# Zaggy1024/RaytracerCore

Hardware: AMD Instinct MI355X
Metric: Mrays/sec (primary+secondary) and samples/sec at 1080p, Cornell box (higher is better)
Workload: dtype f32; 1 GPU; bounce.txt camera 0 1920x1080 x 256 spp per GPU per step; traversal=brute, recursion=10, kernel_build=scene-specialised (hiprtc)

## Files before the change

include/rtcore.h:

```cpp
#ifndef RTCORE_H
#define RTCORE_H

#ifndef __HIPCC_RTC__
#include <stdint.h>
#include <stddef.h>
#endif

#ifdef __cplusplus
extern "C" {
#endif

#define RTCORE_ABI_VERSION 6

typedef enum rt_status {
    RT_OK = 0,
    RT_ERR_ARG = -1,
    RT_ERR_HIP = -2,
    RT_ERR_OOM = -3,
    RT_ERR_NCCL = -4,
    RT_ERR_PARSE = -5,
    RT_ERR_NODEVICE = -6,
    RT_ERR_STATE = -7
} rt_status;

// ... 93 lines not shown
int rt_scene_get_info(const rt_scene* scene, rt_scene_info* info);
void rt_scene_destroy(rt_scene* scene);
int rt_set_bvh_builder(int32_t builder);
int rt_scene_get_build_stats(const rt_scene* scene, double* out, int32_t n);
int rt_set_jit(int32_t on);
int rt_scene_get_jit_error(const rt_scene* scene, char* buf, int32_t cap);
int rt_debug_jit_compile(const char* arch, int32_t grouped, char* log, int32_t cap);
int rt_debug_jit_header(const rt_scene_params* params, const rt_prim* prims, int32_t n_prims, const rt_camera* camera,
                        int32_t grouped, char* buf, int64_t cap);
int rt_scene_check_bvh(rt_scene* scene);
#define RT_LAYOUT_COUNT 10
int rt_debug_brute_layout(const rt_prim* prims, int32_t n_prims, int32_t* out, int32_t n_out);
int rt_debug_item_order(int32_t w, int32_t h, int32_t spp, int32_t chunks, int32_t pool, int32_t band,
                        int32_t band_stride, int32_t band_offset, uint32_t* out, int64_t cap_words, int32_t* info);
int rt_debug_scene_bound(const rt_prim* prims, int32_t n_prims, float* lo, float* hi, float* info);
int rt_debug_ray_log(rt_scene* scene, void* d_log, uint32_t cap, void* d_count);
int rt_debug_vn_rehit(const double* v0, const double* e01, const double* e02, int32_t mirror, double u, double v,
                      const float* dir, int32_t* inside, double* t, double* origin);
int rt_debug_trace_rays(rt_scene* scene, const void* d_rays, uint32_t n, void* d_hits, int32_t waves_per_simd,
                        void* d_stats, void* stream, float* ms);

int rt_render_tile(rt_scene* scene, int32_t x0, int32_t y0, int32_t w, int32_t h, int32_t spp,
                   uint64_t seed, uint64_t sample_base, rt_color* sum_rgb, uint32_t* samples,
                   uint32_t* misses, uint64_t* rays_out);

int rt_render_tile_1spp(rt_scene* scene, int32_t x0, int32_t y0, int32_t w, int32_t h,
                        uint64_t seed, uint64_t sample_index, rt_color* out);

int rt_primary_ids(rt_scene* scene, int32_t x0, int32_t y0, int32_t w, int32_t h, int32_t* ids_out);

// ... 143 lines not shown
```

raytracercore_amd/__init__.py:

```python
from __future__ import annotations

import ctypes as C
import enum
import os
from dataclasses import dataclass
from typing import List, Optional, Sequence, Tuple

import numpy as np

_HERE = os.path.dirname(os.path.abspath(__file__))
LIB_PATH = os.path.join(_HERE, "librtcore_hip.so")
REPO_ROOT = os.path.dirname(_HERE)

RT_OK = 0
ABI_VERSION = 6
RT_PRIM_TRIANGLE, RT_PRIM_SPHERE, RT_PRIM_PLANE = 0, 1, 2
RT_FLAG_MIRROR, RT_FLAG_TWOSIDED, RT_FLAG_INVERT, RT_FLAG_HASNORMALS, RT_FLAG_TRANSFORMED = 1, 2, 4, 8, 16
RT_CAMERA_FRUSTUM, RT_CAMERA_ORTHO = 0, 1
RT_TRAVERSAL_AUTO, RT_TRAVERSAL_BRUTE, RT_TRAVERSAL_BVH, RT_TRAVERSAL_BVH2, RT_TRAVERSAL_GROUPED = 0, 1, 2, 3, 4
RT_BVH_BUILDER_AUTO, RT_BVH_BUILDER_HOST, RT_BVH_BUILDER_GPU = 0, 1, 2
(RT_BOUNCE_SKIPPED, RT_BOUNCE_DIFFUSE, RT_BOUNCE_SPECULAR, RT_BOUNCE_SPECULAR_FAIL, RT_BOUNCE_TRANSMITTED,
 RT_BOUNCE_EMISSION, RT_BOUNCE_PURE_BLACK, RT_BOUNCE_RECURSION_COMPLETE, RT_BOUNCE_MISSED, RT_BOUNCE_DEBUG) = range(10)
BOUNCE_TYPE_NAMES = ("Skipped", "Diffuse", "Specular", "SpecularFail", "Transmitted", "Emission", "PureBlack",
                     "RecursionComplete", "Missed", "Debug")
# ... 187 lines not shown
        "rt_frame_render": (C.c_int, [C.c_void_p, C.c_int32, C.c_uint64, C.c_uint64, P(rt_color), P(C.c_uint32),
                                      P(C.c_uint32), P(C.c_uint64)]),
        "rt_frame_submit": (C.c_int, [C.c_void_p, C.c_int32, C.c_uint64, C.c_uint64]),
        "rt_frame_collect": (C.c_int, [C.c_void_p, P(rt_color), P(C.c_uint32), P(C.c_uint32), P(C.c_uint64)]),
        "rt_frame_inject_fault": (C.c_int, [C.c_void_p, C.c_int32]),
        "rt_frame_destroy": (None, [C.c_void_p]),
        "rt_parse_scene": (C.c_int, [C.c_char_p, P(rt_scene_params), P(rt_prim), P(C.c_int32), P(rt_camera),
                                     P(C.c_int32)]),
        "rt_sample_output": (C.c_int32, [rt_color, C.c_uint32, C.c_uint32, rt_color, C.c_double, C.c_double]),
        "rt_tonemap_device": (C.c_int, [C.c_void_p, C.c_void_p, C.c_void_p, C.c_int32, C.c_int32, rt_color, C.c_double,
                                        C.c_double, C.c_void_p, C.c_void_p]),
        "rt_ref_bvh_export": (C.c_int, [P(rt_prim), C.c_int32, P(C.c_int32), P(C.c_double), P(C.c_int32),
                                        P(C.c_int32)]),
        "rt_debug_item_order": (C.c_int, [C.c_int32] * 8 + [P(C.c_uint32), C.c_int64, P(C.c_int32)]),
        "rt_debug_scene_bound": (C.c_int, [P(rt_prim), C.c_int32, P(C.c_float), P(C.c_float), P(C.c_float)]),
        "rt_debug_ray_log": (C.c_int, [C.c_void_p, C.c_void_p, C.c_uint32, C.c_void_p]),
        "rt_debug_vn_rehit": (C.c_int, [P(C.c_double), P(C.c_double), P(C.c_double), C.c_int32, C.c_double,
                                        C.c_double, P(C.c_float), P(C.c_int32), P(C.c_double), P(C.c_double)]),
        "rt_debug_trace_rays": (C.c_int, [C.c_void_p, C.c_void_p, C.c_uint32, C.c_void_p, C.c_int32, C.c_void_p,
                                          C.c_void_p, P(C.c_float)]),
        "rt_query_rays": (C.c_int, [C.c_void_p, C.c_int32, C.c_void_p, C.c_int64, C.c_void_p]),
        "rt_query_rays_device": (C.c_int, [C.c_void_p, C.c_int32, C.c_void_p, C.c_int64, C.c_void_p, C.c_void_p]),
        "rt_camera_rays": (C.c_int, [P(rt_camera)] + [C.c_int32] * 6 + [C.c_void_p]),
        "rt_select_pixels": (C.c_int, [C.c_void_p, C.c_void_p] + [C.c_int32] * 5 + [C.c_void_p]),
        "rt_select_pixels_device": (C.c_int, [C.c_void_p, C.c_void_p] + [C.c_int32] * 5 + [C.c_void_p, C.c_void_p]),
        "rt_select_rays": (C.c_int, [C.c_void_p, C.c_void_p, C.c_int32, C.c_void_p, C.c_int64, C.c_void_p]),
        "rt_select_rays_device": (C.c_int, [C.c_void_p, C.c_void_p, C.c_int32, C.c_void_p, C.c_int64, C.c_void_p,
                                            C.c_void_p]),
        "rt_debug_select_rays": (C.c_int, [P(rt_prim), C.c_int32, C.c_void_p, C.c_int32, C.c_void_p, C.c_int64,
                                           C.c_void_p]),
# ... 102 lines not shown
    return out[:n], dict(zip(("n_chunks", "chunk", "pool", "n_split"), (int(v) for v in info)))


def scene_bound(prims: Sequence[rt_prim]) -> dict:
    lib = load_library()
    n = len(prims)
    arr = (rt_prim * max(1, n))(*prims)
    lo, hi, info = (C.c_float * 3)(), (C.c_float * 3)(), (C.c_float * 2)()
    state = lib.rt_debug_scene_bound(arr, n, lo, hi, info)
    if state < 0:
        _check(state)
    return {"lo": np.array(lo, np.float32), "hi": np.array(hi, np.float32), "limit": np.float32(info[0]),
            "pad": np.float32(info[1]), "state": int(state)}


def ref_bvh_export(prims: Sequence[rt_prim]) -> Tuple[np.ndarray, np.ndarray, int, int]:
    lib = load_library()
    n = len(prims)
    arr = (rt_prim * max(1, n))(*prims)
    order = np.zeros(max(1, n), np.int32)
    boxes = np.zeros((max(1, 2 * n), 8), np.float64)
    nodes, depth = C.c_int32(0), C.c_int32(0)
    _check(lib.rt_ref_bvh_export(arr, n, order.ctypes.data_as(C.POINTER(C.c_int32)),
                                 boxes.ctypes.data_as(C.POINTER(C.c_double)), C.byref(nodes), C.byref(depth)))
    return order[:n], boxes[:nodes.value], nodes.value, depth.value


def sample_output(sum_rgb: Tuple[float, float, float], samples: int, misses: int,
                  background=(0.0, 0.0, 0.0), background_alpha: float = 0.0, exposure: float = 1.0) -> int:
    lib = load_library()
# ... 114 lines not shown

    def close(self) -> None:
        if self.handle:
            self.lib.rt_scene_destroy(self.handle)
            self.handle = C.c_void_p()

    def __del__(self):
        try:
            self.close()
        except Exception:
            pass

    def set_traversal(self, traversal: int) -> None:
        _check(self.lib.rt_scene_set_traversal(self.handle, traversal))

    def info(self) -> rt_scene_info:
        inf = rt_scene_info()
        _check(self.lib.rt_scene_get_info(self.handle, C.byref(inf)))
        return inf

    def check_bvh(self) -> None:
        _check(self.lib.rt_scene_check_bvh(self.handle))

    def jit_error(self) -> str:
        buf = C.create_string_buffer(4096)
        self.lib.rt_scene_get_jit_error(self.handle, buf, len(buf))
        return buf.value.decode(errors="replace")

    def build_stats(self) -> dict:
        out = (C.c_double * len(BUILD_STAT_NAMES))()
# ... 323 lines not shown
```

raytracercore_amd/csrc/api_debug.hip:

```cpp
#include <cstdlib>
#include <cstring>

#include "rt_scene.h"

namespace {

int n_bvh_prims(const std::vector<HostPrim>& H)
{
    int nb = 0;
    for (const HostPrim& p : H) nb += p.kind != RT_PRIM_PLANE;
    return nb;
}

HostRecords report_records(const std::vector<HostPrim>& H)
{
    const bool host_tree = builder_for(n_bvh_prims(H)) == RT_BVH_BUILDER_HOST;
    return make_host_records(H, host_tree ? grouping_max_leaf(GroupingTree::LayoutReport, (int)H.size(), false) : 0,
                             group_max_default());
}

}

extern "C" {

// ... 422 lines not shown
            set_error("rt_debug_scene_bound: unknown primitive kind at index " + std::to_string(i));
            return RT_ERR_ARG;
        }
    const SceneBound b = make_scene_bound(prepare_prims(prims, n_prims));
    for (int k = 0; k < 3; k++) {
        lo[k] = b.lo[k];
        hi[k] = b.hi[k];
    }
    if (info) {
        info[0] = b.limit;
        info[1] = b.pad;
    }
    return b.empty ? 1 : (b.limit < 0.0f ? 2 : 0);
}

int rt_parse_scene(const char* text, rt_scene_params* params, rt_prim* prims, int32_t* n_prims, rt_camera* cameras,
                   int32_t* n_cameras)
{
    if (!text || !n_prims || !n_cameras) {
        set_error("rt_parse_scene: bad argument");
        return RT_ERR_ARG;
    }
    ParsedScene ps;
    std::string err;
    if (!parse_scene_text(text, ps, err)) {
        set_error(err);
        return RT_ERR_PARSE;
    }
    const int cap_p = *n_prims, cap_c = *n_cameras;
    *n_prims = (int32_t)ps.prims.size();
// ... 45 lines not shown
```

raytracercore_amd/csrc/kernels_path.hip:

```cpp
#include "../../include/rtcore_rng.h"
#include "rt_kernels.h"
#ifdef RT_SCENE_CONST
#include "rt_scene_const.h"
#endif

namespace rtc {
namespace {

struct V3 {
    float x, y, z;
};
__device__ __forceinline__ V3 v3(float x, float y, float z) { return V3{x, y, z}; }
__device__ __forceinline__ V3 xyz(float4 a) { return V3{a.x, a.y, a.z}; }
__device__ __forceinline__ V3 operator+(V3 a, V3 b) { return {a.x + b.x, a.y + b.y, a.z + b.z}; }
__device__ __forceinline__ V3 operator-(V3 a, V3 b) { return {a.x - b.x, a.y - b.y, a.z - b.z}; }
__device__ __forceinline__ V3 operator*(V3 a, float s) { return {a.x * s, a.y * s, a.z * s}; }
__device__ __forceinline__ V3 operator*(V3 a, V3 b) { return {a.x * b.x, a.y * b.y, a.z * b.z}; }
__device__ __forceinline__ V3 operator-(V3 a) { return {-a.x, -a.y, -a.z}; }
__device__ __forceinline__ float dot(V3 a, V3 b) { return fmaf(a.x, b.x, fmaf(a.y, b.y, a.z * b.z)); }
__device__ __forceinline__ bool known_zero(float c)
{
#if defined(RT_SCENE_CONST)
    return __builtin_constant_p(c) && c == 0.0f;
#else
// ... 966 lines not shown
    L.active = true;
    L.item_open = L.live = false;
    L.item = 0;
    L.fx = L.fy = L.s_next = 0;
    L.pkey = rt_key2{0u, 0u};
    L.ar = L.ag = L.ab = 0.0f;
    L.cnt = 0;
    L.pool_next = L.pool_end = 0;
    L.split_j = 0;
}

__device__ __forceinline__ unsigned lanes_below(unsigned long long m)
{
    return __builtin_amdgcn_mbcnt_hi((unsigned)(m >> 32), __builtin_amdgcn_mbcnt_lo((unsigned)m, 0u));
}
template <class ParT>
__device__ __forceinline__ void item_pixel(unsigned item, const ParT& p, int& px, int& py, int& c, int& fx, int& fy)
{
    const unsigned q = item & 63u, t = item >> 6;
    c = (int)(t & (unsigned)(p.n_chunks - 1));
    unsigned by, bx;
    const unsigned blk = t >> p.log2_chunks;
    if (p.magic_bx != 0) {
        by = __umulhi(blk, p.magic_bx);
        bx = blk - by * (unsigned)p.blocks_x;
    } else {
        divmod(blk, (unsigned)p.blocks_x, p.inv_blocks_x, by, bx);
    }
    px = (int)bx * 8 + (int)(q & 7);
    py = (int)by * 8 + (int)(q >> 3);
    fx = p.x0 + px;
    fy = p.y0 + py;
    if (p.band > 0) {
        unsigned bq, br;
        if (p.band_log2 >= 0) {
            bq = (unsigned)py >> p.band_log2;
            br = (unsigned)py & (unsigned)(p.band - 1);
        } else {
// ... 94 lines not shown
                L.active = false;
            } else if constexpr (RAYS) {
                const unsigned ri = item_ray(L.item, p);
                const int s0 = (int)((L.item >> 6) & (unsigned)(p.n_chunks - 1)) * p.chunk;
                if (ri < p.n_rays && s0 < p.spp) {
                    L.item_open = true;
                    if (!NT) L.s_next = s0;
                    L.cnt = (unsigned)(min(p.spp, s0 + p.chunk) - s0) << 16;
                    if (!NT) {
                        L.fx = (int)ri;
                        L.pkey = rt_rng_pixel_key(p.seed_key, p.stream_base + (unsigned long long)ri);
                    }
                }
            } else {
                int px, py, c, fx, fy;
                item_pixel(L.item, p, px, py, c, fx, fy);
                if (px < p.w && py < p.h && c * p.chunk < p.spp) {
                    L.item_open = true;
                    const int s0 = c * p.chunk;
                    if (!NT) L.s_next = s0;
                    L.cnt = (unsigned)(min(p.spp, s0 + p.chunk) - s0) << 16;
                    if (!NT) {
                        L.fx = fx;
                        L.fy = fy;
                    }
                    const unsigned long long pix = (unsigned long long)fy * (unsigned long long)p.scene.width +
                                                   (unsigned long long)fx;
                    if (!NT && p.pkeys) L.pkey = p.pkeys[pix];
                    else if (!NT) L.pkey = rt_rng_pixel_key(p.seed_key, pix);
                }
            }
// ... 200 lines not shown
            test_planes(sc, tests, S.o, S.d, S.prev, b);
            if (VN && __builtin_isnan(S.d.x + S.d.y + S.d.z)) b = Best{__builtin_huge_valf(), -1};
            if (STATS) t2 = __builtin_readcyclecounter();
            bounce<VN, false, false, STATS>(L, S, sc, R, vnormals, tests, pq->prims_d, b, *pq);
        } else if (STATS) {
            t2 = __builtin_readcyclecounter();
        }
        if (STATS) {
            const unsigned long long t3 = __builtin_readcyclecounter();
            cnt.cyc_start += t1 - t0;
            cnt.cyc_trace += t2 - t1;
            cnt.cyc_shade += t3 - t2;
            cnt.iters++;
        }
    }
    flush_counts<STATS>(wave_rays, cnt, *(const ParamsC*)pp, lane);
}

template <bool CULL, bool LDS, bool STATS, bool VN, bool RAYS = false>
__global__ void __launch_bounds__(256, CULL ? RT_GROUPED_WAVES : RT_PATH_WAVES)
    path_kernel(PathScene, const CameraF* __restrict__ camp, const PathParams* __restrict__ pp, const TestRec*,
                const RectRec*, const FrameRec*, const PrimF*, const NodeF*, const Node4Q*, const GroupRec*,
                const XformF*, const MatF*, const float4*)
{
    path_body<CULL, LDS, STATS, VN, RAYS>(camp, pp);
}

template <bool STATS, class GroupP, class RectP, class BoxP>
__device__ __forceinline__ void test_outer(GroupP groups, RectP rects, BoxP boxes, V3 o, V3 d, int prev, Best& b,
                                           unsigned& n_tests)
// ... 599 lines not shown
            break;
        }
        if (walk_step<STACK, true>(w, trav, p.spec, fetch, id, oi, stk, tests, rows, xf, o, d, -1, b, n_tri, n_sph).ended) {
            trav = false;
            if (!P.early && b.sg < 0) outside();
            P.out[idx] = b.sg >= 0 ? 1 : 0;
        }
    }
}

__global__ void accumulate_kernel(PathParams p, double* sum, uint32_t* samples, uint32_t* misses, size_t plane)
{
    const int x = blockIdx.x * 16 + (threadIdx.x & 15);
    const int y = blockIdx.y * 16 + (threadIdx.x >> 4);
    if (x >= p.w || y >= p.h) return;
    const size_t blk = (size_t)((y >> 3) * p.blocks_x + (x >> 3));
    const int q = (y & 7) * 8 + (x & 7);
    const size_t i = (size_t)y * p.w + x;
    double r = sum[i], g = sum[plane + i], bl = sum[2 * plane + i];
    uint32_t ns = 0, nm = 0;
    const int used = (p.spp + p.chunk - 1) / p.chunk;
    for (int c = 0; c < used; c++) {
        const float4 v = p.partial[(((blk << p.log2_chunks) + c) << 6) + q];
        r += v.x;
        g += v.y;
        bl += v.z;
        const uint32_t k = __float_as_uint(v.w);
        ns += k & 0xFFFFu;
        nm += k >> 16;
    }
    sum[i] = r;
    sum[plane + i] = g;
    sum[2 * plane + i] = bl;
// ... 68 lines not shown
    const double bam = nm / total, bk = bam * back_alpha;
    r += (br - r) * bk;
    g += (bg - g) * bk;
    b += (bb - b) * bk;
    a += (back_alpha - a) * bam;
    const double gamma = 1 / 2.2;
    argb[i] = (int32_t)color_code(pow(r, gamma), pow(g, gamma), pow(b, gamma), a);
}

__global__ void colors_1spp_kernel(PathParams p, float* __restrict__ out)
{
    const size_t npix = (size_t)p.w * p.h;
    const size_t o = (size_t)blockIdx.x * blockDim.x + threadIdx.x;
    if (o >= npix) return;
    const int x = (int)(o / (size_t)p.h), y = (int)(o - (size_t)x * p.h);
    const int q = ((y >> 3) * p.blocks_x + (x >> 3)) * 64 + (y & 7) * 8 + (x & 7);
    const float4 v = p.partial[q];
    const bool miss = (__float_as_uint(v.w) & 0xFFFFu) == 0;
    out[3 * o + 0] = miss ? -1.0f : v.x;
    out[3 * o + 1] = miss ? -1.0f : v.y;
    out[3 * o + 2] = miss ? -1.0f : v.z;
}

__global__ void trace_host_layout_kernel(int w, int h, int spp, int rows, const float4* __restrict__ rays,
                                         const float4* __restrict__ samples, float4* __restrict__ rays_out,
                                         float4* __restrict__ samples_out)
{
    const size_t n = (size_t)w * h * spp;
    const size_t i = (size_t)blockIdx.x * blockDim.x + threadIdx.x;
    if (i >= n * (size_t)(rows + 1)) return;
    const size_t so = i / (size_t)(rows + 1), row = i - so * (size_t)(rows + 1);
    const size_t pix = so / (size_t)spp, k = so - pix * (size_t)spp;
// ... 385 lines not shown
```

raytracercore_amd/csrc/launch_params.cpp:

```cpp
#include "launch_params.h"

#include <algorithm>
#include <cmath>
#include <cstdlib>

#include "host_scene.h"

namespace rtc {

void set_item_order(PathParams& p)
{
    const char* e = getenv("RTCORE_ITEM_ORDER");
    bool dense = !(e && e[0] == '0');
    const unsigned slots = (unsigned)p.pool / 64u;
    const unsigned used = (unsigned)((p.spp + p.chunk - 1) / p.chunk);
    const unsigned n_blocks = (unsigned)(p.n_pad / 64);
    for (;; dense = false) {
        const unsigned n_real = dense ? used : (unsigned)p.n_chunks;
        const unsigned n_full = dense && p.spp % p.chunk != 0 ? used - 1 : n_real;
        p.tpb = n_full / slots;
        p.tail_first = p.tpb * (unsigned)p.pool;
        p.tail_len = (n_real - p.tpb * slots) * 64u;
        p.magic_tpb = 0;
        if (p.tpb <= 1) break;
        const uint64_t M = ((1ull << 32) + p.tpb - 1) / p.tpb;
        const uint64_t err = M * p.tpb - (1ull << 32);
        if (M < (1ull << 32) && (uint64_t)n_blocks * p.tpb * err < (1ull << 32)) {
            p.magic_tpb = (unsigned)M;
            break;
        }
    }
    p.linear = p.tail_len == 0 && p.tpb * slots == (unsigned)p.n_chunks;
    for (int g = 0; g < kMaxSplit; g++) {
        const unsigned b = g < p.n_split ? (p.split_start[g + 1] - p.split_start[g]) >> (p.log2_chunks + 6) : 0u;
        p.split_full[g] = b * p.tpb;
        p.split_tickets[g] = p.split_full[g] + (p.tail_len ? b : 0u);
    }
}

PathParams make_params_for(int kernel, int chunks_over, int pool_over, int x0, int y0, int w, int h, int spp,
                           uint64_t seed, uint64_t base, double chunk_npix)
{
    PathParams p{};
    p.x0 = x0;
    p.y0 = y0;
    p.w = w;
    p.h = h;
    p.band = 0;
    p.spp = spp;
    const int base_chunks = kernel >= 2 ? 64 : 24;
    int chunks = base_chunks;
    const double npix = chunk_npix > 0.0 ? chunk_npix : (double)w * (double)h;
// ... 19 lines not shown
        if (M < (1ull << 32) && max_blk * err < (1ull << 32)) p.magic_bx = (unsigned)M;
    }
    int pool_mul = kernel == 0 ? 1 : 2;
    if (const char* e = getenv("RTCORE_POOL_MUL")) pool_mul = std::max(1, std::min(64, atoi(e)));
    if (pool_over > 0) pool_mul = std::max(1, std::min(64, pool_over / 64));
    p.pool = 64;
    while (p.pool < 64 * pool_mul && p.pool < 64 * p.n_chunks) p.pool *= 2;
    p.batch = kernel < 2 ? 64 : 0;
    if (const char* e = getenv("RTCORE_ITEM_BATCH")) p.batch = std::max(0, std::min(64, atoi(e)));
    p.scene_bound = 1;
    if (const char* e = getenv("RTCORE_SCENE_BOUND")) p.scene_bound = atoi(e) != 0 ? 1 : 0;
    p.refill = 28;
    if (const char* e = getenv("RTCORE_BVH_REFILL")) p.refill = std::max(1, std::min(64, atoi(e)));
    p.spec = 12;
    if (const char* e = getenv("RTCORE_BVH_SPEC")) p.spec = std::max(1, std::min(64, atoi(e)));
    p.n_split = 1;
    const int n_blocks = p.n_pad / 64;
    int want = kMaxSplit;
    if (const char* e = getenv("RTCORE_XCD_SPLIT")) want = atoi(e) > 0 ? kMaxSplit : 1;
    if (want > 1 && n_blocks >= 4 * kMaxSplit) p.n_split = kMaxSplit;
    for (int g = 0; g <= p.n_split; g++)
        p.split_start[g] = (unsigned)((int64_t)n_blocks * g / p.n_split) * (unsigned)(p.n_chunks * 64);
    set_item_order(p);
    p.seed = seed;
    p.seed_key = rt_rng_seed_key(seed);
    p.sample_base = base;
    return p;
}

PathParams make_params_rays(int kernel, int64_t n, int spp, uint64_t seed, uint64_t base, uint64_t stream_base)
{
    PathParams p = make_params_for(kernel, 0, 0, 0, 0, 8, (int)((n + 7) / 8), spp, seed, base, 2073600.0);
    p.n_rays = (unsigned)n;
    p.stream_base = stream_base;
    return p;
}

int64_t render_rays_max_n(int kernel, int spp)
// ... 70 lines not shown
```

raytracercore_amd/csrc/launch_params.h:

```cpp
#pragma once
#include "rt_kernels.h"

namespace rtc {

PathParams make_params_for(int kernel, int chunks_over, int pool_over, int x0, int y0, int w, int h, int spp,
                           uint64_t seed, uint64_t base, double chunk_npix);
PathParams make_params_rays(int kernel, int64_t n, int spp, uint64_t seed, uint64_t base, uint64_t stream_base);
int64_t render_rays_max_n(int kernel, int spp);
void set_item_order(PathParams& p);
void set_band(PathParams& p, int band, int stride, int offset);
int64_t list_tickets(const PathParams& p, uint32_t* out, int64_t cap_words);

int band_set_rows(int H, int band, int stride, int offset);
int band_slot_rows(int H, int band, int stride);
void scatter_band_set(const unsigned char* slot, size_t plane, int W, int H, int band, int stride, int offset,
                      rt_color* sum_rgb, uint32_t* samples, uint32_t* misses);

}
```

raytracercore_amd/csrc/rt_kernels.h:

```cpp
#pragma once
#include "../../include/rtcore_rng.h"
#include "rt_internal.h"

namespace rtc {

constexpr int kMaxSplit = 8;
constexpr int kSplitStride = 32;

struct PathParams {
    int x0, y0, w, h;
    int band, band_stride, band_offset;
    int band_log2;
    float inv_band;
    int spp;
    int chunk;
    int n_chunks;
    int log2_chunks;
    int blocks_x;
    int n_pad;
    int refill;
    int spec;
    int pool;
    float inv_blocks_x;
    unsigned magic_bx;
// ... 27 lines not shown
    const Node4Q* nodes4;
    const XformF* xf;
    const MatF* mats;
    const float4* vnormals;
    const PrimD* prims_d;
    float4* ray_log;
    unsigned int* ray_log_n;
    unsigned int ray_log_cap;
    float4* rec_rays;
    float4* rec_samples;
    unsigned int rec_max;
    const double2* ray_list;
    unsigned int n_rays;
    unsigned long long stream_base;
    int scene_bound;
};
constexpr int kRecRows = 6;

template <class ParT>
__host__ __device__ inline void ticket_items(const ParT& p, unsigned g, unsigned t, unsigned& first, unsigned& len)
{
    const unsigned full = p.split_full[g];
    unsigned blk, off;
    if (t < full) {
        blk = p.magic_tpb ? (unsigned)(((unsigned long long)t * p.magic_tpb) >> 32) : t;
        off = (t - blk * p.tpb) * (unsigned)p.pool;
        len = (unsigned)p.pool;
    } else {
        blk = t - full;
        off = p.tail_first;
        len = p.tail_len;
// ... 105 lines not shown
```

raytracercore_amd/csrc/rt_scene.h:

```cpp
#pragma once
#include <algorithm>
#include <array>
#include <functional>
#include <string>
#include <vector>

#include "host_scene.h"
#include "launch_params.h"
#include "rt_jit.h"
#include "rt_kernels.h"
#include "scene_records.h"

using namespace rtc;

#define HIP_TRY(expr)                                                                                  \
    do {                                                                                                \
        hipError_t e_ = (expr);                                                                         \
        if (e_ != hipSuccess) {                                                                         \
            set_error(std::string(#expr) + ": " + hipGetErrorString(e_));                               \
            return e_ == hipErrorOutOfMemory ? RT_ERR_OOM : RT_ERR_HIP;                                 \
        }                                                                                               \
    } while (0)

template <class T>
// ... 155 lines not shown
    unsigned int* ray_log_n = nullptr;
    unsigned int ray_log_cap = 0;
    int stats_blocks_per_cu = 1;
    DevBuf<unsigned long long> stats_buf;
    bool tracing = false;
    DevBuf<unsigned long long> trace_stats;
    DevBuf<float4> trace_rays, trace_samples, trace_out;
    CameraD camd{};
    CameraF camf{};
    DevBuf<CameraF> camf_d;
    static constexpr int kParamRing = 256;
    DevBuf<PathParams> params_d;
    PathParams* params_h = nullptr;
    std::array<hipEvent_t, kParamRing> slot_ev{};
    unsigned params_next = 0;
    bool has_camera = false;
    bool flat_overflow = false;
    hipStream_t stream = nullptr;
    static constexpr int kTimeRing = 64;
    std::array<hipEvent_t, kTimeRing> t_start{}, t_end{};
    uint64_t launches = 0;
    hipEvent_t done_ev = nullptr;
    hipStream_t last_stream = nullptr;
    bool any_op = false;
    uint64_t device_bytes = 0;

    ~rt_scene()
    {
        if (jit.fn) jit_release(device, jit.fn);
        if (params_h) (void)hipHostFree(params_h);
        for (hipEvent_t e : slot_ev)
            if (e) (void)hipEventDestroy(e);
        if (done_ev) (void)hipEventDestroy(done_ev);
        for (hipEvent_t e : copy_ev)
            if (e) (void)hipEventDestroy(e);
        for (hipEvent_t e : band_ev)
            if (e) (void)hipEventDestroy(e);
        for (hipEvent_t e : query_up_ev)
            if (e) (void)hipEventDestroy(e);
        if (copy_stream) {
            (void)hipStreamSynchronize(copy_stream);
            (void)hipStreamDestroy(copy_stream);
        }
        for (int i = 0; i < kTimeRing; i++) {
            if (t_start[i]) (void)hipEventDestroy(t_start[i]);
            if (t_end[i]) (void)hipEventDestroy(t_end[i]);
        }
        if (stream) (void)hipStreamDestroy(stream);
// ... 32 lines not shown
```

raytracercore_amd/csrc/rtcore_api.hip:

```cpp
#include <atomic>
#include <chrono>
#include <cmath>
#include <cstring>
#include <memory>

#include "rt_scene.h"

namespace rtc {
static thread_local std::string g_error;
void set_error(const std::string& msg) { g_error = msg; }
}

extern "C" {

int rt_set_jit(int32_t on)
{
    if (on != 0 && on != 1) {
        set_error("rt_set_jit: on must be 0 or 1");
        return RT_ERR_ARG;
    }
    jit_set_enabled(on == 1);
    return RT_OK;
}

// ... 115 lines not shown
    if (!s || !cam || (cam->kind != RT_CAMERA_FRUSTUM && cam->kind != RT_CAMERA_ORTHO)) {
        set_error("rt_scene_set_camera: bad argument");
        return RT_ERR_ARG;
    }
    HIP_TRY(hipSetDevice(s->device));
    camera_init(*cam, s->params.width, s->params.height, s->camd, s->camf);
    HIP_TRY(hipDeviceSynchronize());
    HIP_TRY(s->camf_d.reserve(1));
    HIP_TRY(hipMemcpy(s->camf_d.p, &s->camf, sizeof(CameraF), hipMemcpyHostToDevice));
    if (s->groups_gr_host.size() > 1 && !getenv("RTCORE_NO_GROUP_SORT")) {
        const std::vector<GroupRec> g = groups_nearest_first(s->groups_gr_host, s->camd);
        HIP_TRY(hipMemcpy(s->grouped_d.groups.p, g.data(), g.size() * sizeof(GroupRec), hipMemcpyHostToDevice));
        s->grouped_h.groups = g;
    }
    s->has_camera = true;
    s->jit_gen++;
    const int rc = calibrate_grouping(s);
    if (rc == RT_OK) (void)prepare_jit(s);
    return rc;
}

int rt_scene_set_traversal(rt_scene* s, int32_t traversal)
{
    if (!s || traversal < RT_TRAVERSAL_AUTO || traversal > RT_TRAVERSAL_GROUPED) {
        set_error("rt_scene_set_traversal: bad argument");
        return RT_ERR_ARG;
    }
    HIP_TRY(hipSetDevice(s->device));
    const int before = s->traversal;
    s->traversal = traversal;
// ... 391 lines not shown
```

raytracercore_amd/csrc/scene_upload.hip:

```cpp
#include <atomic>
#include <cmath>
#include <cstdio>
#include <cstdlib>
#include <cstring>
#include <unordered_map>

#include "bvh_gpu.h"
#include "rt_scene.h"

namespace rtc {

static std::atomic<int> g_builder{RT_BVH_BUILDER_AUTO};
constexpr int kGpuBuildMin = 1 << 22;

int builder_for(int n_bvh)
{
    int b = g_builder.load();
    if (b == RT_BVH_BUILDER_AUTO)
        if (const char* e = getenv("RTCORE_BVH_BUILDER"))
            b = std::strcmp(e, "gpu") == 0 ? RT_BVH_BUILDER_GPU : std::strcmp(e, "host") == 0 ? RT_BVH_BUILDER_HOST : b;
    if (b == RT_BVH_BUILDER_AUTO) b = n_bvh >= kGpuBuildMin ? RT_BVH_BUILDER_GPU : RT_BVH_BUILDER_HOST;
    return n_bvh > 0 ? b : RT_BVH_BUILDER_HOST;
}

// ... 506 lines not shown
    if (!s->params_h) {
        HIP_TRY(hipHostMalloc(&s->params_h, sizeof(PathParams) * rt_scene::kParamRing, hipHostMallocDefault));
        HIP_TRY(s->params_d.reserve(rt_scene::kParamRing));
    }
    const unsigned slot = s->params_next++ % rt_scene::kParamRing;
    hipEvent_t& sev = s->slot_ev[slot];
    if (sev) HIP_TRY(hipEventSynchronize(sev));
    else HIP_TRY(hipEventCreateWithFlags(&sev, hipEventDisableTiming));
    s->params_h[slot] = p;
    HIP_TRY(hipMemcpyAsync(s->params_d.p + slot, s->params_h + slot, sizeof(PathParams), hipMemcpyHostToDevice, stream));
    HIP_TRY(hipEventRecord(sev, stream));
    *d_out = s->params_d.p + slot;
    return RT_OK;
}

int run_path(rt_scene* s, PathParams& p, unsigned long long* d_rays, hipStream_t stream, bool timed)
{
    const size_t need = (size_t)p.n_chunks * (size_t)p.n_pad;
    uint64_t tickets = 0;
    for (int g = 0; g < p.n_split; g++) tickets += p.split_tickets[g];
    if (need > 0xF0000000ull || tickets > need / 64) {
        set_error("tile x spp too large for one launch; split the tile");
        return RT_ERR_ARG;
    }
    HIP_TRY(s->partial.reserve(need));
    HIP_TRY(s->counter.reserve(kMaxSplit * kSplitStride));
    p.partial = s->partial.p;
    p.counter = s->counter.p;
    p.rays = d_rays;
    p.stats = s->stats_on ? (s->tracing ? s->trace_stats.p : s->stats_buf.p) : nullptr;
    p.ray_log = (s->stats_on && !s->tracing && s->variant >= 4) ? s->ray_log : nullptr;
    p.ray_log_n = s->ray_log_n;
    p.ray_log_cap = s->ray_log_cap;
    if (p.ray_log) s->ray_log = nullptr;
    if (s->any_op && stream != s->last_stream) HIP_TRY(hipStreamWaitEvent(stream, s->done_ev, 0));
    HIP_TRY(hipMemsetAsync(p.counter, 0, sizeof(unsigned int) * kSplitStride * p.n_split, stream));
    int grid = s->n_cu * (s->stats_on ? s->stats_blocks_per_cu : s->blocks_per_cu);
    p.stack_ovf = nullptr;
    if (s->variant >= 4) {
        HIP_TRY(s->stack_ovf.reserve((size_t)grid * 256 * kStackOverflow));
        p.stack_ovf = s->stack_ovf.p;
    }
    const int jit = s->tracing ? 0 : prepare_jit(s);
    int jit_grid = jit ? s->n_cu * s->jit.blocks_per_cu : 0;
    if ((s->variant >> 1) < 2 && !s->stats_on) {
        constexpr double kSamplesPerLane = 6.0;
        const double samples = (double)p.w * (double)p.h * (double)p.spp;
        int cap = (int)std::ceil(samples / ((double)s->n_cu * 256.0 * kSamplesPerLane));
        if (const char* e = getenv("RTCORE_GRID_BPC")) cap = atoi(e);
        cap = std::max(1, cap);
        if (jit) jit_grid = s->n_cu * std::min(s->jit.blocks_per_cu, cap);
        else grid = s->n_cu * std::min(s->blocks_per_cu, cap);
    }
    const int tslot = (int)(s->launches % rt_scene::kTimeRing);
    if (timed) HIP_TRY(hipEventRecord(s->t_start[tslot], stream));
    fill_launch(s->dev, s->variant, p);
    p.pkeys = nullptr;
    static const bool pkeys_on = !(getenv("RTCORE_PIXEL_KEYS") && getenv("RTCORE_PIXEL_KEYS")[0] == '0');
    if ((s->variant >> 1) < 2 && !s->stats_on && pkeys_on) {
        if (!s->pkeys_valid || s->pkeys_seed != p.seed) {
            HIP_TRY(s->pkeys.reserve((size_t)s->params.width * (size_t)s->params.height));
            HIP_TRY(launch_pixel_keys(p.seed_key, s->params.width, s->params.height, s->pkeys.p, stream));
// ... 100 lines not shown
```

Before: 109,300 Mrays/s.

## Cull screen blocks whose rays cannot hit the projected scene bound

Measured after the change: 118,000 Mrays/s (median of 6 runs). 1.08x the previous value.

```diff
diff --git a/include/rtcore.h b/include/rtcore.h
--- a/include/rtcore.h
+++ b/include/rtcore.h
@@ -131,6 +131,9 @@
 int rt_debug_item_order(int32_t w, int32_t h, int32_t spp, int32_t chunks, int32_t pool, int32_t band,
                         int32_t band_stride, int32_t band_offset, uint32_t* out, int64_t cap_words, int32_t* info);
 int rt_debug_scene_bound(const rt_prim* prims, int32_t n_prims, float* lo, float* hi, float* info);
+int rt_debug_block_cull(const rt_prim* prims, int32_t n_prims, const rt_camera* camera, int32_t width, int32_t height,
+                        int32_t x0, int32_t y0, int32_t w, int32_t h, int32_t band, int32_t band_stride,
+                        int32_t band_offset, uint8_t* dead, int64_t cap, int32_t* info);
 int rt_debug_ray_log(rt_scene* scene, void* d_log, uint32_t cap, void* d_count);
 int rt_debug_vn_rehit(const double* v0, const double* e01, const double* e02, int32_t mirror, double u, double v,
                       const float* dir, int32_t* inside, double* t, double* origin);
diff --git a/raytracercore_amd/__init__.py b/raytracercore_amd/__init__.py
--- a/raytracercore_amd/__init__.py
+++ b/raytracercore_amd/__init__.py
@@ -225,6 +225,8 @@
                                         P(C.c_int32)]),
         "rt_debug_item_order": (C.c_int, [C.c_int32] * 8 + [P(C.c_uint32), C.c_int64, P(C.c_int32)]),
         "rt_debug_scene_bound": (C.c_int, [P(rt_prim), C.c_int32, P(C.c_float), P(C.c_float), P(C.c_float)]),
+        "rt_debug_block_cull": (C.c_int, [P(rt_prim), C.c_int32, P(rt_camera)] + [C.c_int32] * 9 +
+                                [P(C.c_uint8), C.c_int64, P(C.c_int32)]),
         "rt_debug_ray_log": (C.c_int, [C.c_void_p, C.c_void_p, C.c_uint32, C.c_void_p]),
         "rt_debug_vn_rehit": (C.c_int, [P(C.c_double), P(C.c_double), P(C.c_double), C.c_int32, C.c_double,
                                         C.c_double, P(C.c_float), P(C.c_int32), P(C.c_double), P(C.c_double)]),
@@ -357,6 +359,27 @@
             "pad": np.float32(info[1]), "state": int(state)}
 
 
+def block_cull(prims: Sequence[rt_prim], camera: rt_camera, size: Tuple[int, int],
+               window: Optional[Tuple[int, int, int, int]] = None,
+               bands: Optional[Tuple[int, int, int]] = None) -> Tuple[np.ndarray, int]:
+    lib = load_library()
+    n = len(prims)
+    arr = (rt_prim * max(1, n))(*prims)
+    cam = rt_camera.from_buffer_copy(camera)
+    b = bands or (0, 0, 0)
+    W, H = size
+    rows = lib.rt_band_rows(H, b[0], b[1], b[2]) if bands else H
+    x0, y0, w, h = window or (0, 0, W, rows)
+    bx, by = (w + 7) // 8, (h + 7) // 8
+    dead = np.zeros(max(1, bx * by), np.uint8)
+    info = (C.c_int32 * 2)()
+    live = lib.rt_debug_block_cull(arr, n, C.byref(cam), W, H, x0, y0, w, h, b[0], b[1], b[2],
+                                   dead.ctypes.data_as(C.POINTER(C.c_uint8)), bx * by, info)
+    if live < 0:
+        _check(live)
+    return dead[:bx * by].reshape(by, bx).astype(bool), int(live)
+
+
 def ref_bvh_export(prims: Sequence[rt_prim]) -> Tuple[np.ndarray, np.ndarray, int, int]:
     lib = load_library()
     n = len(prims)
@@ -501,6 +524,10 @@
     def set_traversal(self, traversal: int) -> None:
         _check(self.lib.rt_scene_set_traversal(self.handle, traversal))
 
+    def set_camera(self, camera: rt_camera) -> None:
+        self.camera = rt_camera.from_buffer_copy(camera)
+        _check(self.lib.rt_scene_set_camera(self.handle, C.byref(self.camera)))
+
     def info(self) -> rt_scene_info:
         inf = rt_scene_info()
         _check(self.lib.rt_scene_get_info(self.handle, C.byref(inf)))
diff --git a/raytracercore_amd/csrc/api_debug.hip b/raytracercore_amd/csrc/api_debug.hip
--- a/raytracercore_amd/csrc/api_debug.hip
+++ b/raytracercore_amd/csrc/api_debug.hip
@@ -460,6 +460,41 @@
     return b.empty ? 1 : (b.limit < 0.0f ? 2 : 0);
 }
 
+int rt_debug_block_cull(const rt_prim* prims, int32_t n_prims, const rt_camera* camera, int32_t width, int32_t height,
+                        int32_t x0, int32_t y0, int32_t w, int32_t h, int32_t band, int32_t band_stride,
+                        int32_t band_offset, uint8_t* dead, int64_t cap, int32_t* info)
+{
+    const bool banded = band > 0;
+    if (n_prims < 0 || (n_prims > 0 && !prims) || !camera || width <= 0 || height <= 0 || w <= 0 || h <= 0 || x0 < 0 ||
+        y0 < 0 || x0 + w > width || cap < 0 || (cap > 0 && !dead) || band < 0 ||
+        (camera->kind != RT_CAMERA_FRUSTUM && camera->kind != RT_CAMERA_ORTHO) ||
+        (banded && (band_stride <= 0 || band_offset < 0 || band_offset >= band_stride)) || (!banded && y0 + h > height)) {
+        set_error("rt_debug_block_cull: bad argument");
+        return RT_ERR_ARG;
+    }
+    int n_planes = 0;
+    for (int i = 0; i < n_prims; i++) {
+        if (prims[i].kind < 0 || prims[i].kind > 2) {
+            set_error("rt_debug_block_cull: unknown primitive kind at index " + std::to_string(i));
+            return RT_ERR_ARG;
+        }
+        n_planes += prims[i].kind == RT_PRIM_PLANE ? 1 : 0;
+    }
+    const SceneBound b = make_scene_bound(prepare_prims(prims, n_prims));
+    CameraD camd;
+    CameraF camf;
+    camera_init(*camera, width, height, camd, camf);
+    const CullWindow win{x0, y0, w, h, banded ? band : 0, banded ? band_stride : 0, banded ? band_offset : 0};
+    std::vector<unsigned char> flags;
+    const int live = cull_blocks(camf, b, n_planes, win, flags);
+    for (size_t i = 0; i < flags.size() && (int64_t)i < cap; i++) dead[i] = flags[i];
+    if (info) {
+        info[0] = (w + 7) / 8;
+        info[1] = (h + 7) / 8;
+    }
+    return live;
+}
+
 int rt_parse_scene(const char* text, rt_scene_params* params, rt_prim* prims, int32_t* n_prims, rt_camera* cameras,
                    int32_t* n_cameras)
 {
diff --git a/raytracercore_amd/csrc/block_cull.cpp b/raytracercore_amd/csrc/block_cull.cpp
--- /dev/null
+++ b/raytracercore_amd/csrc/block_cull.cpp
@@ -0,0 +1,177 @@
+#include "block_cull.h"
+
+#include <algorithm>
+#include <cmath>
+
+namespace rtc {
+
+namespace {
+
+constexpr double kMargin = 0.25;
+constexpr double kAhead = 1e-3;
+
+struct P2 {
+    double x, y;
+};
+
+struct Hull {
+    std::vector<P2> v;
+    double xmin, xmax, ymin, ymax;
+};
+
+double cross2(P2 o, P2 a, P2 b) { return (a.x - o.x) * (b.y - o.y) - (a.y - o.y) * (b.x - o.x); }
+
+void convex_hull(std::vector<P2> pts, Hull& h)
+{
+    std::sort(pts.begin(), pts.end(), [](P2 a, P2 b) { return a.x < b.x || (a.x == b.x && a.y < b.y); });
+    std::vector<P2> v(2 * pts.size());
+    size_t k = 0;
+    for (size_t i = 0; i < pts.size(); i++) {
+        while (k >= 2 && cross2(v[k - 2], v[k - 1], pts[i]) <= 0.0) k--;
+        v[k++] = pts[i];
+    }
+    for (size_t i = pts.size() - 1, t = k + 1; i > 0; i--) {
+        while (k >= t && cross2(v[k - 2], v[k - 1], pts[i - 1]) <= 0.0) k--;
+        v[k++] = pts[i - 1];
+    }
+    v.resize(k > 1 ? k - 1 : k);
+    h.v = v;
+    h.xmin = h.ymin = INFINITY;
+    h.xmax = h.ymax = -INFINITY;
+    for (P2 p : pts) {
+        h.xmin = std::min(h.xmin, p.x);
+        h.xmax = std::max(h.xmax, p.x);
+        h.ymin = std::min(h.ymin, p.y);
+        h.ymax = std::max(h.ymax, p.y);
+    }
+}
+
+bool separated(const Hull& h, double xa, double xb, double ya, double yb)
+{
+    if (xb < h.xmin || xa > h.xmax || yb < h.ymin || ya > h.ymax) return true;
+    const size_t n = h.v.size();
+    if (n < 3) return false;
+    for (size_t i = 0; i < n; i++) {
+        const P2 p = h.v[i], q = h.v[i + 1 == n ? 0 : i + 1];
+        const double nx = q.y - p.y, ny = -(q.x - p.x);
+        const double cx = nx > 0.0 ? xa : xb, cy = ny > 0.0 ? ya : yb;
+        if (nx * (cx - p.x) + ny * (cy - p.y) > 0.0) return true;
+    }
+    return false;
+}
+
+struct V3d {
+    double x, y, z;
+};
+V3d crs(V3d a, V3d b) { return {a.y * b.z - a.z * b.y, a.z * b.x - a.x * b.z, a.x * b.y - a.y * b.x}; }
+double dot(V3d a, V3d b) { return a.x * b.x + a.y * b.y + a.z * b.z; }
+V3d v3d(const float4& f) { return {(double)f.x, (double)f.y, (double)f.z}; }
+
+bool project_bound(const CameraF& c, const SceneBound& b, int frame_w, Hull& hull)
+{
+    const bool frustum = c.kind == RT_CAMERA_FRUSTUM;
+    const double vals[] = {c.position.x, c.position.y, c.position.z, c.look.x, c.look.y, c.look.z, c.side.x,
+                           c.side.y, c.side.z, c.up.x, c.up.y, c.up.z, c.w2, c.h2, c.tan_x, c.tan_y,
+                           c.h_mult, c.v_mult, c.image_plane, c.dof, c.focal_length, c.tan_x_per_px, c.tan_y_per_px};
+    for (double v : vals)
+        if (!std::isfinite(v)) return false;
+    if (c.dof != 0.0f) return false;
+    const V3d pos = v3d(c.position), look = v3d(c.look), side = v3d(c.side), up = v3d(c.up);
+    const double apos = std::fabs(pos.x) + std::fabs(pos.y) + std::fabs(pos.z);
+    const V3d da = crs(up, look), db = crs(look, side), dc = crs(side, up);
+    const double det = dot(side, da);
+    if (!(std::fabs(det) > 0.5 && std::fabs(det) < 2.0)) return false;
+    const double sxa = frustum ? c.tan_x_per_px : c.h_mult, sya = frustum ? c.tan_y_per_px : c.v_mult;
+    if (sxa == 0.0 || sya == 0.0) return false;
+    const double scale = std::min(std::fabs(sxa), std::fabs(sya));
+    if (frustum) {
+        if (!(apos <= (double)b.limit)) return false;
+    } else {
+        const double reach = std::fabs((double)c.w2 * c.h_mult) * (std::fabs(side.x) + std::fabs(side.y) + std::fabs(side.z)) +
+                             std::fabs((double)c.h2 * c.v_mult) * (std::fabs(up.x) + std::fabs(up.y) + std::fabs(up.z));
+        if (!(apos + 2.0 * reach + std::fabs((double)c.image_plane) <= (double)b.limit)) return false;
+    }
+    std::vector<P2> pts;
+    double c_min = INFINITY, c_max = 0.0;
+    for (int k = 0; k < 8; k++) {
+        const V3d P = {(k & 1) ? (double)b.hi[0] + b.pad : (double)b.lo[0] - b.pad,
+                       (k & 2) ? (double)b.hi[1] + b.pad : (double)b.lo[1] - b.pad,
+                       (k & 4) ? (double)b.hi[2] + b.pad : (double)b.lo[2] - b.pad};
+        const V3d v = {P.x - pos.x, P.y - pos.y, P.z - pos.z};
+        const double a = dot(v, da) / det, bb = dot(v, db) / det, cc = dot(v, dc) / det;
+        if (!(cc > kAhead * std::sqrt(dot(v, v))) || !(cc > 0.0)) return false;
+        c_min = std::min(c_min, cc);
+        c_max = std::max(c_max, cc);
+        if (frustum) pts.push_back({(a / cc + (double)c.tan_x) / sxa, (bb / cc + (double)c.tan_y) / sya});
+        else pts.push_back({a / sxa + (double)c.w2, bb / sya + (double)c.h2});
+    }
+    double err;
+    if (frustum) {
+        const double L = 1.0 + std::fabs((double)c.tan_x) + std::fabs((double)c.tan_y);
+        err = std::ldexp(L * L, -20) / scale +
+              std::ldexp(apos + std::fabs((double)c.image_plane), -22) / (c_min * scale);
+    } else {
+        const double R = apos + std::fabs((double)c.w2 * c.h_mult) + std::fabs((double)c.h2 * c.v_mult) +
+                         std::fabs((double)c.image_plane);
+        err = std::ldexp(R + c_max, -22) / scale + std::ldexp((double)std::max(frame_w, 1), -22);
+    }
+    if (!(err <= kMargin / 8.0)) return false;
+    for (P2 p : pts)
+        if (!(std::isfinite(p.x) && std::isfinite(p.y))) return false;
+    convex_hull(pts, hull);
+    return true;
+}
+
+}
+
+int cull_blocks(const CameraF& cam, const SceneBound& bound, int n_planes, const CullWindow& win,
+                std::vector<unsigned char>& dead)
+{
+    const int bxn = (win.w + 7) / 8, byn = (win.h + 7) / 8;
+    const int n = bxn * byn;
+    dead.assign((size_t)n, 0);
+    if (n_planes > 0) return n;
+    if (bound.empty) {
+        dead.assign((size_t)n, 1);
+        return 0;
+    }
+    if (!(bound.limit >= 0.0f)) return n;
+    Hull hull;
+    if (!project_bound(cam, bound, (int)(2.0f * cam.w2), hull)) return n;
+    int live = 0;
+    for (int by = 0; by < byn; by++) {
+        int run_a[8], run_b[8], runs = 0;
+        for (int py = by * 8; py < std::min(win.h, by * 8 + 8); py++) {
+            int fy = win.y0 + py;
+            if (win.band > 0) fy = win.y0 + ((py / win.band) * win.band_stride + win.band_offset) * win.band + py % win.band;
+            if (runs > 0 && fy == run_b[runs - 1] + 1) run_b[runs - 1] = fy;
+            else {
+                run_a[runs] = run_b[runs] = fy;
+                runs++;
+            }
+        }
+        for (int bx = 0; bx < bxn; bx++) {
+            const double xa = (double)(win.x0 + bx * 8) - kMargin;
+            const double xb = (double)(win.x0 + std::min(win.w, bx * 8 + 8)) + kMargin;
+            bool is_dead = true;
+            for (int r = 0; r < runs && is_dead; r++)
+                is_dead = separated(hull, xa, xb, (double)run_a[r] - kMargin, (double)(run_b[r] + 1) + kMargin);
+            dead[(size_t)by * bxn + bx] = is_dead ? 1 : 0;
+            live += is_dead ? 0 : 1;
+        }
+    }
+    return live;
+}
+
+uint64_t dead_pixels(const CullWindow& win, const std::vector<unsigned char>& dead)
+{
+    const int bxn = (win.w + 7) / 8, byn = (win.h + 7) / 8;
+    uint64_t n = 0;
+    for (int by = 0; by < byn; by++)
+        for (int bx = 0; bx < bxn; bx++)
+            if (dead[(size_t)by * bxn + bx])
+                n += (uint64_t)(std::min(win.w, bx * 8 + 8) - bx * 8) * (uint64_t)(std::min(win.h, by * 8 + 8) - by * 8);
+    return n;
+}
+
+}
diff --git a/raytracercore_amd/csrc/block_cull.h b/raytracercore_amd/csrc/block_cull.h
--- /dev/null
+++ b/raytracercore_amd/csrc/block_cull.h
@@ -0,0 +1,19 @@
+#pragma once
+#include <cstdint>
+#include <vector>
+
+#include "rt_internal.h"
+
+namespace rtc {
+
+struct CullWindow {
+    int x0, y0, w, h;
+    int band, band_stride, band_offset;
+};
+
+int cull_blocks(const CameraF& cam, const SceneBound& bound, int n_planes, const CullWindow& win,
+                std::vector<unsigned char>& dead);
+
+uint64_t dead_pixels(const CullWindow& win, const std::vector<unsigned char>& dead);
+
+}
diff --git a/raytracercore_amd/csrc/kernels_path.hip b/raytracercore_amd/csrc/kernels_path.hip
--- a/raytracercore_amd/csrc/kernels_path.hip
+++ b/raytracercore_amd/csrc/kernels_path.hip
@@ -1004,14 +1004,18 @@
 {
     return __builtin_amdgcn_mbcnt_hi((unsigned)(m >> 32), __builtin_amdgcn_mbcnt_lo((unsigned)m, 0u));
 }
-template <class ParT>
+template <bool TABLE = false, class ParT>
 __device__ __forceinline__ void item_pixel(unsigned item, const ParT& p, int& px, int& py, int& c, int& fx, int& fy)
 {
     const unsigned q = item & 63u, t = item >> 6;
     c = (int)(t & (unsigned)(p.n_chunks - 1));
     unsigned by, bx;
     const unsigned blk = t >> p.log2_chunks;
-    if (p.magic_bx != 0) {
+    if (TABLE && p.cull != nullptr) {
+        const unsigned v = p.cull[kCullTable + blk];
+        bx = v & 0xFFFFu;
+        by = v >> 16;
+    } else if (p.magic_bx != 0) {
         by = __umulhi(blk, p.magic_bx);
         bx = blk - by * (unsigned)p.blocks_x;
     } else {
@@ -1136,7 +1140,7 @@
                 }
             } else {
                 int px, py, c, fx, fy;
-                item_pixel(L.item, p, px, py, c, fx, fy);
+                item_pixel<!NT>(L.item, p, px, py, c, fx, fy);
                 if (px < p.w && py < p.h && c * p.chunk < p.spp) {
                     L.item_open = true;
                     const int s0 = c * p.chunk;
@@ -1367,6 +1371,8 @@
             cnt.iters++;
         }
     }
+    if (!STATS && !RAYS && P0.cull != nullptr && blockIdx.x == 0 && threadIdx.x < 64)
+        wave_rays += ((unsigned long long)P0.cull[0] | (unsigned long long)P0.cull[1] << 32) * (unsigned long long)P0.spp;
     flush_counts<STATS>(wave_rays, cnt, *(const ParamsC*)pp, lane);
 }
 
@@ -1996,9 +2002,17 @@
     const int x = blockIdx.x * 16 + (threadIdx.x & 15);
     const int y = blockIdx.y * 16 + (threadIdx.x >> 4);
     if (x >= p.w || y >= p.h) return;
-    const size_t blk = (size_t)((y >> 3) * p.blocks_x + (x >> 3));
+    size_t blk = (size_t)((y >> 3) * p.blocks_x + (x >> 3));
     const int q = (y & 7) * 8 + (x & 7);
     const size_t i = (size_t)y * p.w + x;
+    if (p.cull) {
+        const int live = (int)p.cull[kCullTable + (p.n_pad >> 6) + blk];
+        if (live < 0) {
+            misses[i] += (uint32_t)p.spp;
+            return;
+        }
+        blk = (size_t)live;
+    }
     double r = sum[i], g = sum[plane + i], bl = sum[2 * plane + i];
     uint32_t ns = 0, nm = 0;
     const int used = (p.spp + p.chunk - 1) / p.chunk;
@@ -2097,8 +2111,10 @@
     const size_t o = (size_t)blockIdx.x * blockDim.x + threadIdx.x;
     if (o >= npix) return;
     const int x = (int)(o / (size_t)p.h), y = (int)(o - (size_t)x * p.h);
-    const int q = ((y >> 3) * p.blocks_x + (x >> 3)) * 64 + (y & 7) * 8 + (x & 7);
-    const float4 v = p.partial[q];
+    int blk = (y >> 3) * p.blocks_x + (x >> 3);
+    if (p.cull) blk = (int)p.cull[kCullTable + (p.n_pad >> 6) + blk];
+    const int q = (blk < 0 ? 0 : blk) * 64 + (y & 7) * 8 + (x & 7);
+    const float4 v = blk < 0 ? make_float4(0.0f, 0.0f, 0.0f, 0.0f) : p.partial[q];
     const bool miss = (__float_as_uint(v.w) & 0xFFFFu) == 0;
     out[3 * o + 0] = miss ? -1.0f : v.x;
     out[3 * o + 1] = miss ? -1.0f : v.y;
diff --git a/raytracercore_amd/csrc/launch_params.cpp b/raytracercore_amd/csrc/launch_params.cpp
--- a/raytracercore_amd/csrc/launch_params.cpp
+++ b/raytracercore_amd/csrc/launch_params.cpp
@@ -36,6 +36,18 @@
         p.split_full[g] = b * p.tpb;
         p.split_tickets[g] = p.split_full[g] + (p.tail_len ? b : 0u);
     }
+}
+
+void set_blocks(PathParams& p, int n_blocks)
+{
+    p.n_pad = n_blocks * 64;
+    p.n_split = 1;
+    int want = kMaxSplit;
+    if (const char* e = getenv("RTCORE_XCD_SPLIT")) want = atoi(e) > 0 ? kMaxSplit : 1;
+    if (want > 1 && n_blocks >= 4 * kMaxSplit) p.n_split = kMaxSplit;
+    for (int g = 0; g <= p.n_split; g++)
+        p.split_start[g] = (unsigned)((int64_t)n_blocks * g / p.n_split) * (unsigned)(p.n_chunks * 64);
+    set_item_order(p);
 }
 
 PathParams make_params_for(int kernel, int chunks_over, int pool_over, int x0, int y0, int w, int h, int spp,
@@ -85,14 +97,7 @@
     if (const char* e = getenv("RTCORE_BVH_REFILL")) p.refill = std::max(1, std::min(64, atoi(e)));
     p.spec = 12;
     if (const char* e = getenv("RTCORE_BVH_SPEC")) p.spec = std::max(1, std::min(64, atoi(e)));
-    p.n_split = 1;
-    const int n_blocks = p.n_pad / 64;
-    int want = kMaxSplit;
-    if (const char* e = getenv("RTCORE_XCD_SPLIT")) want = atoi(e) > 0 ? kMaxSplit : 1;
-    if (want > 1 && n_blocks >= 4 * kMaxSplit) p.n_split = kMaxSplit;
-    for (int g = 0; g <= p.n_split; g++)
-        p.split_start[g] = (unsigned)((int64_t)n_blocks * g / p.n_split) * (unsigned)(p.n_chunks * 64);
-    set_item_order(p);
+    set_blocks(p, p.n_pad / 64);
     p.seed = seed;
     p.seed_key = rt_rng_seed_key(seed);
     p.sample_base = base;
diff --git a/raytracercore_amd/csrc/launch_params.h b/raytracercore_amd/csrc/launch_params.h
--- a/raytracercore_amd/csrc/launch_params.h
+++ b/raytracercore_amd/csrc/launch_params.h
@@ -8,6 +8,7 @@
 PathParams make_params_rays(int kernel, int64_t n, int spp, uint64_t seed, uint64_t base, uint64_t stream_base);
 int64_t render_rays_max_n(int kernel, int spp);
 void set_item_order(PathParams& p);
+void set_blocks(PathParams& p, int n_blocks);
 void set_band(PathParams& p, int band, int stride, int offset);
 int64_t list_tickets(const PathParams& p, uint32_t* out, int64_t cap_words);
 
diff --git a/raytracercore_amd/csrc/rt_kernels.h b/raytracercore_amd/csrc/rt_kernels.h
--- a/raytracercore_amd/csrc/rt_kernels.h
+++ b/raytracercore_amd/csrc/rt_kernels.h
@@ -65,7 +65,9 @@
     unsigned int n_rays;
     unsigned long long stream_base;
     int scene_bound;
+    const unsigned int* cull;
 };
+constexpr int kCullTable = 4;
 constexpr int kRecRows = 6;
 
 template <class ParT>
diff --git a/raytracercore_amd/csrc/rt_scene.h b/raytracercore_amd/csrc/rt_scene.h
--- a/raytracercore_amd/csrc/rt_scene.h
+++ b/raytracercore_amd/csrc/rt_scene.h
@@ -5,6 +5,7 @@
 #include <string>
 #include <vector>
 
+#include "block_cull.h"
 #include "host_scene.h"
 #include "launch_params.h"
 #include "rt_jit.h"
@@ -193,6 +194,20 @@
     PathParams* params_h = nullptr;
     std::array<hipEvent_t, kParamRing> slot_ev{};
     unsigned params_next = 0;
+    struct CullEntry {
+        bool valid = false;
+        unsigned cam_gen = 0;
+        CullWindow win{};
+        int n_live = 0, n_blocks = 0;
+        uint64_t dead_px = 0, used = 0;
+        DevBuf<unsigned int> dev;
+        HostBuf<unsigned int> host;
+        hipEvent_t up = nullptr;
+    };
+    static constexpr int kCullEntries = 4;
+    std::array<CullEntry, kCullEntries> cull_cache;
+    uint64_t cull_clock = 0;
+    unsigned cam_gen = 0;
     bool has_camera = false;
     bool flat_overflow = false;
     hipStream_t stream = nullptr;
@@ -211,6 +226,8 @@
         for (hipEvent_t e : slot_ev)
             if (e) (void)hipEventDestroy(e);
         if (done_ev) (void)hipEventDestroy(done_ev);
+        for (CullEntry& c : cull_cache)
+            if (c.up) (void)hipEventDestroy(c.up);
         for (hipEvent_t e : copy_ev)
             if (e) (void)hipEventDestroy(e);
         for (hipEvent_t e : band_ev)
diff --git a/raytracercore_amd/csrc/rtcore_api.hip b/raytracercore_amd/csrc/rtcore_api.hip
--- a/raytracercore_amd/csrc/rtcore_api.hip
+++ b/raytracercore_amd/csrc/rtcore_api.hip
@@ -153,6 +153,7 @@
         s->grouped_h.groups = g;
     }
     s->has_camera = true;
+    s->cam_gen++;
     s->jit_gen++;
     const int rc = calibrate_grouping(s);
     if (rc == RT_OK) (void)prepare_jit(s);
diff --git a/raytracercore_amd/csrc/scene_upload.hip b/raytracercore_amd/csrc/scene_upload.hip
--- a/raytracercore_amd/csrc/scene_upload.hip
+++ b/raytracercore_amd/csrc/scene_upload.hip
@@ -544,8 +544,77 @@
     return RT_OK;
 }
 
+constexpr int kCullMinBlocks = 4096;
+static int plan_block_cull(rt_scene* s, const PathParams& p, rt_scene::CullEntry*& ent, bool& fresh)
+{
+    ent = nullptr;
+    fresh = false;
+    if ((s->variant >> 1) >= 2 || s->stats_on || s->tracing) return RT_OK;
+    if (const char* e = getenv("RTCORE_BLOCK_CULL"))
+        if (atoi(e) == 0) return RT_OK;
+    int min_blocks = kCullMinBlocks;
+    if (const char* e = getenv("RTCORE_BLOCK_CULL_MIN")) min_blocks = std::max(1, atoi(e));
+    const int n_blocks = p.n_pad / 64;
+    if (n_blocks < min_blocks || p.blocks_x > 0xFFFF || n_blocks / p.blocks_x > 0xFFFF) return RT_OK;
+    const CullWindow win{p.x0, p.y0, p.w, p.h, p.band > 0 ? p.band : 0, p.band > 0 ? p.band_stride : 0,
+                         p.band > 0 ? p.band_offset : 0};
+    auto same = [](const CullWindow& a, const CullWindow& b) {
+        return a.x0 == b.x0 && a.y0 == b.y0 && a.w == b.w && a.h == b.h && a.band == b.band &&
+               a.band_stride == b.band_stride && a.band_offset == b.band_offset;
+    };
+    rt_scene::CullEntry* c = nullptr;
+    for (rt_scene::CullEntry& e : s->cull_cache)
+        if (e.valid && e.cam_gen == s->cam_gen && same(e.win, win)) c = &e;
+    if (!c) {
+        auto age = [&](const rt_scene::CullEntry& e) { return e.valid && e.cam_gen == s->cam_gen ? e.used : 0; };
+        c = &s->cull_cache[0];
+        for (rt_scene::CullEntry& e : s->cull_cache)
+            if (age(e) < age(*c)) c = &e;
+        c->valid = false;
+        if (c->up) HIP_TRY(hipEventSynchronize(c->up));
+        else HIP_TRY(hipEventCreateWithFlags(&c->up, hipEventDisableTiming));
+        std::vector<unsigned char> dead;
+        c->n_live = cull_blocks(s->camf, s->dev.bound, s->dev.n_pln, win, dead);
+        c->n_blocks = n_blocks;
+        c->dead_px = dead_pixels(win, dead);
+        c->cam_gen = s->cam_gen;
+        c->win = win;
+        if (c->n_live < n_blocks) {
+            const size_t words = (size_t)kCullTable + (size_t)c->n_live + (size_t)n_blocks;
+            HIP_TRY(c->host.reserve(words));
+            HIP_TRY(c->dev.reserve(words));
+            unsigned int* h = c->host.p;
+            h[0] = (unsigned)(c->dead_px & 0xFFFFFFFFull);
+            h[1] = (unsigned)(c->dead_px >> 32);
+            h[2] = (unsigned)c->n_live;
+            h[3] = (unsigned)n_blocks;
+            unsigned live = 0;
+            for (int b = 0; b < n_blocks; b++) {
+                if (!dead[(size_t)b]) h[kCullTable + live] = (unsigned)(b % p.blocks_x) | (unsigned)(b / p.blocks_x) << 16;
+                h[kCullTable + c->n_live + b] = dead[(size_t)b] ? 0xFFFFFFFFu : live;
+                live += dead[(size_t)b] ? 0u : 1u;
+            }
+            fresh = true;
+        } else {
+            c->valid = true;
+        }
+    }
+    c->used = ++s->cull_clock;
+    if (c->n_live < c->n_blocks) ent = c;
+    return RT_OK;
+}
+
 int run_path(rt_scene* s, PathParams& p, unsigned long long* d_rays, hipStream_t stream, bool timed)
 {
+    rt_scene::CullEntry* cull = nullptr;
+    bool cull_fresh = false;
+    p.cull = nullptr;
+    const int crc = plan_block_cull(s, p, cull, cull_fresh);
+    if (crc != RT_OK) return crc;
+    if (cull) {
+        set_blocks(p, cull->n_live);
+        p.cull = cull->dev.p;
+    }
     const size_t need = (size_t)p.n_chunks * (size_t)p.n_pad;
     uint64_t tickets = 0;
     for (int g = 0; g < p.n_split; g++) tickets += p.split_tickets[g];
@@ -564,6 +633,12 @@
     p.ray_log_cap = s->ray_log_cap;
     if (p.ray_log) s->ray_log = nullptr;
     if (s->any_op && stream != s->last_stream) HIP_TRY(hipStreamWaitEvent(stream, s->done_ev, 0));
+    if (cull && cull_fresh) {
+        const size_t words = (size_t)kCullTable + (size_t)cull->n_live + (size_t)cull->n_blocks;
+        HIP_TRY(hipMemcpyAsync(cull->dev.p, cull->host.p, words * sizeof(unsigned int), hipMemcpyHostToDevice, stream));
+        HIP_TRY(hipEventRecord(cull->up, stream));
+        cull->valid = true;
+    }
     HIP_TRY(hipMemsetAsync(p.counter, 0, sizeof(unsigned int) * kSplitStride * p.n_split, stream));
     int grid = s->n_cu * (s->stats_on ? s->stats_blocks_per_cu : s->blocks_per_cu);
     p.stack_ovf = nullptr;
@@ -575,7 +650,7 @@
     int jit_grid = jit ? s->n_cu * s->jit.blocks_per_cu : 0;
     if ((s->variant >> 1) < 2 && !s->stats_on) {
         constexpr double kSamplesPerLane = 6.0;
-        const double samples = (double)p.w * (double)p.h * (double)p.spp;
+        const double samples = ((double)p.w * (double)p.h - (cull ? (double)cull->dead_px : 0.0)) * (double)p.spp;
         int cap = (int)std::ceil(samples / ((double)s->n_cu * 256.0 * kSamplesPerLane));
         if (const char* e = getenv("RTCORE_GRID_BPC")) cap = atoi(e);
         cap = std::max(1, cap);
```
